# kasvii/GATOR

Hardware: AMD Instinct MI355X
Metric: meshes/sec (B=256, J=17) GATOR forward (higher is better)
Workload: dtype f32; 1 GPU; B=256 synthetic Human3.6M 17-joint poses per GPU, GAT+MDR forward fp32; batch_per_gpu=256, global_batch=256, num_joint=17, impl=fused, parallelism=dp1, mode=gather

## Files before the change

gator_amd/csrc/fused_api.hip:

```cpp
#include <hip/hip_runtime.h>

#include <algorithm>
#include <cmath>
#include <cstdlib>
#include <type_traits>
#include <vector>

#include "fused_state.h"
#include "x3_common.h"

namespace gator {
namespace {

static void graph_slot_free(FusedState::GraphSlot& g) {
    if (g.exec) (void)hipGraphExecDestroy((hipGraphExec_t)g.exec);
    if (g.graph) (void)hipGraphDestroy((hipGraph_t)g.graph);
    g.exec = g.graph = nullptr;
}
static void graphs_clear(FusedState* f) {
    for (auto& g : f->graphs) graph_slot_free(g);
    f->graphs.clear();
}
struct WsScope {
    FusedState* f; FusedWs* prev;
    WsScope(FusedState* f_, int i) : f(f_), prev(f_->ws) { f->ws = &f->sets[i]; }
    ~WsScope() { f->ws = prev; }
};

int fused_ensure_ws(gator_ctx* c, int B) {
    FusedState* f = c->fused;
    FusedWs& w = *f->ws;
    if (w.base && B <= w.cap) return GATOR_OK;
    if (w.base) {
        GATOR_HIP_CHECK(hipDeviceSynchronize());
        graphs_clear(f);
    }
    const int cap = B, MT = (cap + 31) / 32, J = c->J;
    const size_t tiles = (size_t)cap * kVT * 2 * kTile;
    size_t n = 0;
    auto layout = [&](float* block) {
        n = 0;
        auto region = [&](auto*& member, size_t floats) {
            if (block) member = reinterpret_cast<std::remove_reference_t<decltype(member)>>(block + n);
            n += (floats + 63) & ~(size_t)63;
        };
        region(w.vcp, (size_t)MT * 3 * kCB * kTile); region(w.vc, (size_t)cap * kV * 3);
        region(w.vf, 3 * tiles); region(w.q, 9 * tiles / 2); region(w.k, 9 * tiles / 2); region(w.v, 9 * tiles / 2);
        region(w.jkv, (size_t)cap * 12 * kTile); region(w.hf, (size_t)cap * kV * 32); region(w.lbf, (size_t)cap * kV * kE);
        region(w.feat, (size_t)cap * J * kC); region(w.vcp3, std::max(upsample_x3_vcp_elems(cap), upsample_x2_vcp_elems(cap)) / 2);
        region(w.lpart, gat_tail_part_floats(cap, J)); region(w.mdr_ctr, mdr_ctr_words(cap)); region(w.hpart, (size_t)cap * kVT * 128);
    };
    layout(nullptr);
    GATOR_TRY(w.base.alloc(n * sizeof(float)));
    GATOR_HIP_CHECK(hipMemset(w.base, 0, n * sizeof(float)));
    GATOR_HIP_CHECK(hipDeviceSynchronize());
    w.cap = cap;
    layout(w.base);
    return GATOR_OK;
}

std::vector<float> d2h(const float* p, size_t n) {
    std::vector<float> v(n);
    (void)hipMemcpy(v.data(), p, n * sizeof(float), hipMemcpyDeviceToHost);
    return v;
}

template <class F>
void fill_tile(float* dst, F tab) {
    for (int g = 0; g < 4; ++g)
        for (int lane = 0; lane < 64; ++lane)
            for (int j = 0; j < 4; ++j) dst[(g * 64 + lane) * 4 + j] = tab(lane & 31, 8 * g + 4 * (lane >> 5) + j);
}

int read_fused_options(const gator_ctx* c, FusedOptions* o) {
    auto flag = [](const char* name, bool dflt) { const char* e = getenv(name); return e ? atoi(e) != 0 : dflt; };
    auto num = [](const char* name, int dflt) { const char* e = getenv(name); return e ? atoi(e) : dflt; };
    auto set = [](const char* name) { return getenv(name) != nullptr; };
    const bool exact = c->arithmetic == GATOR_ARITH_EXACT_SPLIT;
    o->gat_x3 = flag("GATOR_GAT_X3", true);
    o->gat8 = o->gat_x3 && flag("GATOR_GAT8", true);
    o->gat8_h4 = !exact && flag("GATOR_GAT8_H4", true);
    o->gat8_lobyte = o->gat8 && o->gat8_h4 && flag("GATOR_GAT8_LOBYTE", true);
    o->gat_tiled_h4 = !exact && flag("GATOR_GAT_TILED_H4", true);
    o->gat_tiled = num("GATOR_GAT_TILED", -1);
    if (const int m = num("GATOR_GAT_TILED_MIN_BATCH", 0); m > 0) o->gat_tiled_min_batch = m;
    o->mdr_x3 = exact ? 1 : num("GATOR_MDR_X3", 2);
    o->up_x3 = exact ? 1 : num("GATOR_UPSAMPLE_X3", 2);
    if (c->parts & GATOR_PART_MDR) {
        if (o->up_x3 < 0 || o->up_x3 > 2) return fail(GATOR_EINVAL, "GATOR_UPSAMPLE_X3 must be 0, 1 or 2");
        if (o->mdr_x3 < 0 || o->mdr_x3 > 2) return fail(GATOR_EINVAL, "GATOR_MDR_X3 must be 0, 1 or 2");
    }
    o->gat8_tail = o->gat8 && o->gat8_h4 && o->mdr_x3 == 2 && flag("GATOR_GAT8_TAIL", true);
    o->mdr_persist = set("GATOR_MDR_PERSIST") ? flag("GATOR_MDR_PERSIST", false) : -1;
    o->mdr_persist_chunk = num("GATOR_MDR_PERSIST_CHUNK", 0);
    o->mdr_persist_grid = num("GATOR_MDR_PERSIST_GRID", 0);
    o->mdr_head_partials = flag("GATOR_MDR_HEAD_PARTIALS", true);
    o->c3_mdr = o->mdr_x3 == 2 && flag("GATOR_C3_MDR", true);
    o->c3_encoder = o->gat8 && o->gat8_h4 && o->gat_tiled_h4 && flag("GATOR_C3_ENCODER", true);
    o->c3_up_w1 = flag("GATOR_C3_UPSAMPLE_W1", true);
    o->c3_up_bf16 = o->up_x3 != 2 || flag("GATOR_C3_UPSAMPLE_BF16", false);
    o->c3_guard = flag("GATOR_C3_GUARD", true);
    o->graph = flag("GATOR_GRAPH", false);
    o->subbatch_streams = num("GATOR_SUBBATCH_STREAMS", 0);
#ifdef GATOR_DIAG
    o->gat8_dbg = num("GATOR_GAT8_DBG", 0);
    o->gat_stamps = set("GATOR_GAT_STAMPS");
    o->mdr_cut = num("GATOR_MDR_CUT", 0);
    o->mdr_stamps = set("GATOR_MDR_STAMPS");
    o->mdr_solo = set("GATOR_MDR_SOLO");
    o->mdr_ends = set("GATOR_MDR_ENDS");
#endif
    return GATOR_OK;
}

static double sym_eig_max(std::vector<double>& A, int n) {
    for (int sweep = 0; sweep < 64; ++sweep) {
        double off = 0, all = 0;
        for (int p = 0; p < n; ++p)
            for (int q = 0; q < n; ++q) { all += A[p * n + q] * A[p * n + q]; if (q > p) off += A[p * n + q] * A[p * n + q]; }
        if (!(off > 1e-30 * all)) break;
        for (int p = 0; p < n; ++p)
            for (int q = p + 1; q < n; ++q) {
                const double apq = A[p * n + q];
                if (apq == 0) continue;
                const double th = (A[q * n + q] - A[p * n + p]) / (2 * apq);
                const double t = (th >= 0 ? 1.0 : -1.0) / (std::fabs(th) + std::sqrt(th * th + 1));
                const double cs = 1 / std::sqrt(t * t + 1), sn = t * cs;
                for (int k = 0; k < n; ++k) {
                    const double kp = A[k * n + p], kq = A[k * n + q];
                    A[k * n + p] = cs * kp - sn * kq; A[k * n + q] = sn * kp + cs * kq;
                }
                for (int k = 0; k < n; ++k) {
                    const double pk = A[p * n + k], qk = A[q * n + k];
                    A[p * n + k] = cs * pk - sn * qk; A[q * n + k] = sn * pk + cs * qk;
                }
            }
    }
    double m = 0;
    for (int i = 0; i < n; ++i) m = std::max(m, A[i * n + i]);
    return m;
}

float c3_logit_bound(const Weights& w) {
    double worst = 0;
    for (int li = 0; li < 3; ++li) {
        const MdrLayerW& r = w.lay[li];
        const std::vector<float> wq = d2h(r.sa_w[0], 64 * 64), wk = d2h(r.sa_w[1], 64 * 64), bq = d2h(r.sa_b[0], 64), bk = d2h(r.sa_b[1], 64),
                                 a2 = d2h(r.a2, 64), b2 = d2h(r.b2, 64);
        double amax = 0, bn = 0;
        for (int i = 0; i < 64; ++i) { amax = std::max(amax, (double)std::fabs(a2[i])); bn += (double)b2[i] * b2[i]; }
        const double xn = amax * std::sqrt(63.0) + std::sqrt(bn);
        auto head_norm = [&](const std::vector<float>& W, const std::vector<float>& bias, int hd) {
            std::vector<double> G(32 * 32);
            double bb = 0;
            for (int i = 0; i < 32; ++i) {
                bb += (double)bias[32 * hd + i] * bias[32 * hd + i];
                for (int j = 0; j < 32; ++j) {
                    double acc = 0;
                    for (int k = 0; k < 64; ++k) acc += (double)W[(32 * hd + i) * 64 + k] * (double)W[(32 * hd + j) * 64 + k];
                    G[i * 32 + j] = acc;
                }
            }
            return std::sqrt(std::max(sym_eig_max(G, 32), 0.0)) * xn + std::sqrt(bb);
        };
        for (int hd = 0; hd < 2; ++hd)
            worst = std::max(worst, head_norm(wq, bq, hd) * head_norm(wk, bk, hd) / std::sqrt(32.0) * 1.4426950408889634);
    }
    return (float)worst;
}

struct PackItem { const float* src; int64_t wsn, wsk; int N, K; const float** dst; };
template <size_t n>
int pack_linears(const PackItem (&items)[n], float*& p, void* stream) {
    for (const PackItem& it : items) {
        GATOR_TRY(fused_pack_linear(it.src, it.wsn, it.wsk, it.N, it.K, p, stream));
        *it.dst = p;
        p += (size_t)nblk32(it.N) * nblk32(it.K) * kTile;
    }
    return GATOR_OK;
}

int fused_create_gat(gator_ctx* c, FusedState* f, void* stream) {
    const Weights& w = c->w;
    const int J = c->J;
    const size_t blk_tiles = 48 + 16 + 16 + 16 + 16 + 4 + 20 + 64 + 64 + 4 + 4 + 1 + 1;
    const size_t total = (kDepth * blk_tiles + 8 + 2 + 8 + 4 + 12) * kTile;
    GATOR_TRY(f->gbuf.alloc(total * sizeof(float)));
    float* p = f->gbuf;
    auto take = [&](size_t tiles) { float* r = p; p += tiles * kTile; return r; };
    std::vector<float> host;
    auto upload = [&](const std::vector<float>& v) -> const float* {
        float* d = take(v.size() / kTile);
        (void)hipMemcpy(d, v.data(), v.size() * sizeof(float), hipMemcpyHostToDevice);
        return d;
    };
    const std::vector<float> adiag = d2h(c->adj_diag, (size_t)kDepth * J), aoff = d2h(c->adj_off, (size_t)kDepth * J * J),
                             m1 = d2h(c->mask1, (size_t)J * J), m2 = d2h(c->mask2, (size_t)J * J), hb = d2h(c->hop_bias, (size_t)kH * J * J);
    for (int i = 0; i < kDepth; ++i) {
        const GatBlockW& r = w.blk[i];
        GatBlockPk& q = f->gblk[i];
        const PackItem items[] = {
            {r.qkv_w, 128, 1, 384, 128, &q.qkv}, {r.proj_w, 128, 1, 128, 128, &q.proj},
            {r.gcn_W, 1, 128, 128, 128, &q.w0}, {r.gcn_W + 128 * 128, 1, 128, 128, 128, &q.w1},
            {r.xl0_w, 128, 1, 128, 128, &q.lin0}, {r.xl1_w, 128, 1, 16, 128, &q.lin1}, {r.xlb_w, 144, 1, 128, 144, &q.back},
            {r.fc1_w, 128, 1, 512, 128, &q.fc1}, {r.fc2_w, 512, 1, 128, 512, &q.fc2}};
        GATOR_TRY(pack_linears(items, p, stream));
        const std::vector<float> M = d2h(r.gcn_M, (size_t)J * kC), b1 = d2h(r.xl1_b, 16);
        std::vector<float> mc(4 * kTile), md(4 * kTile);
        for (int nb = 0; nb < 4; ++nb) {
            for (int g = 0; g < 4; ++g)
                for (int lane = 0; lane < 64; ++lane)
                    for (int j = 0; j < 4; ++j) {
                        const int tok = 8 * g + 4 * (lane >> 5) + j, n = 32 * nb + (lane & 31);
                        mc[((nb * 4 + g) * 64 + lane) * 4 + j] = tok < J ? M[(size_t)tok * kC + n] : 0.f;
                    }
            fill_tile(md.data() + (size_t)nb * kTile, [&](int t, int ch) { return t < J ? adiag[i * J + t] * M[(size_t)t * kC + 32 * nb + ch] : 0.f; });
        }
        q.mc = upload(mc);
        q.mdT = upload(md);
        std::vector<float> t1(kTile), t2(kTile);
        fill_tile(t1.data(), [&](int t, int j) { return (t < J && j < J) ? aoff[((size_t)i * J + t) * J + j] : 0.f; });
        q.aoffT = upload(t1);
        fill_tile(t2.data(), [&](int t, int ch) {
            if (t >= J || ch >= 16) return 0.f;
            float deg = 0.f;
            for (int j = 0; j < J; ++j) deg += m2[(size_t)t * J + j];
            return deg * b1[ch];
        });
        q.f1b = upload(t2);
    }
    if (f->opt.gat_x3) {
        const int64_t ntiles = (p - f->gblk[0].qkv) / kTile;
        GATOR_TRY(f->gxbuf.alloc((size_t)ntiles * kTileX3 * sizeof(float)));
        int rc = fused_repack_x3(f->gblk[0].qkv, f->gxbuf, ntiles, stream);
        if (rc) return rc;
        if (f->opt.gat_tiled_h4) {
            float left = 0.f;
            GATOR_TRY(f->gxbuf_h3.alloc((size_t)ntiles * kTileX3 * sizeof(float)));
            rc = fused_repack_h3(f->gblk[0].qkv, f->gxbuf_h3, ntiles, &f->gat_tiled_wshift, &left, stream, (int64_t)blk_tiles, 264);
            if (rc == GATOR_OK && left > 1e-7f) rc = fail(GATOR_EUNSUPPORTED, "GAT weights span more than fp16 x 3 planes hold exactly: use GATOR_GAT_TILED_H4=0");
            if (rc) return rc;
        }
        if (f->opt.gat8) {
            rc = gat8_build_stream(f, stream);
            if (rc) return rc;
        }
    }
    std::vector<float> bt(8 * kTile), mt(kTile);
    for (int hd = 0; hd < kH; ++hd)
        fill_tile(bt.data() + (size_t)hd * kTile, [&](int t, int j) { return (t < J && j < J) ? hb[((size_t)hd * J + t) * J + j] : 0.f; });
    f->g_biasT = upload(bt);
    fill_tile(mt.data(), [&](int t, int j) { return (t < J && j < J) ? m1[(size_t)t * J + j] : 0.f; });
    f->g_m1T = upload(mt);
    fill_tile(mt.data(), [&](int t, int j) { return (t < J && j < J) ? m2[(size_t)t * J + j] : 0.f; });
    f->g_m2T = upload(mt);
    {
        std::vector<float> vv((size_t)kDepth * 2048);
        for (int i = 0; i < kDepth; ++i) {
            const GatBlockW& r = w.blk[i];
            const struct { const float* p; int n; } parts[] = {{r.n1w, 128}, {r.n1b, 128}, {r.qkv_b, 384}, {r.proj_b, 128}, {r.gcn_bias, 128},
                                                               {r.xl0_b, 128}, {r.xlb_b, 128}, {r.n2w, 128}, {r.n2b, 128}, {r.fc1_b, 512}, {r.fc2_b, 128}};
            size_t off = (size_t)i * 2048;
            for (auto& pt : parts) {
                const std::vector<float> h = d2h(pt.p, pt.n);
                std::copy(h.begin(), h.end(), vv.begin() + off);
                off += pt.n;
            }
        }
        f->g_vecs = upload(vv);
    }
    {
        float* dst = take(8);
        int rc = fused_pack_linear(w.gl3_W, 64, 1, 128, 64, dst, stream);
        if (rc) return rc;
        f->g_gl3 = dst;
        const std::vector<float> pe = d2h(c->pos_embed, (size_t)J * kC);
        std::vector<float> pt(4 * kTile);
        for (int kb = 0; kb < 4; ++kb)
            fill_tile(pt.data() + (size_t)kb * kTile, [&](int t, int ch) { return t < J ? pe[(size_t)t * kC + 32 * kb + ch] : 0.f; });
        f->g_posT = upload(pt);
    }
    {
        int rc = gat_prepare_device();
        if (rc == GATOR_OK) rc = gat_tiled_prepare_device();
        if (rc == GATOR_OK) rc = gat8_prepare_device();
        if (rc) return rc;
        hipDeviceProp_t prop;
        if (hipGetDeviceProperties(&prop, c->device) == hipSuccess && prop.multiProcessorCount > 0) f->n_cu = prop.multiProcessorCount;
    }
    GATOR_HIP_CHECK(hipStreamSynchronize((hipStream_t)stream));
    GATOR_HIP_CHECK(hipGetLastError());
    return GATOR_OK;
}

}

int fused_create(gator_ctx* c, void* stream) {
    if (c->impl == GATOR_IMPL_BASIC) return GATOR_OK;
    FusedState* f = new FusedState();
    c->fused = f;
    int rc = read_fused_options(c, &f->opt);
    if (rc) return rc;
    f->gat_tiled = f->opt.gat_tiled;
    f->graph_replay = f->opt.graph;
    const Weights& w = c->w;
    if (c->parts & GATOR_PART_GAT) {
        rc = fused_create_gat(c, f, stream);
        if (rc) return rc;
    }
    if (!(c->parts & GATOR_PART_MDR)) return GATOR_OK;
    if (f->opt.c3_mdr) {
        f->c3_logit_bound = c3_logit_bound(w);
        if (f->opt.c3_guard && !(f->c3_logit_bound <= 1024.0f)) f->opt.c3_mdr = f->opt.c3_encoder = false;
    }
    const size_t n_up = f->opt.up_x3 == 0 ? (size_t)3 * kOB * kCB * kTile : 0, n_layer = (size_t)64 * kTile;
    const size_t total = n_up + 3 * n_layer + 24 * kTile + 64 + (size_t)kVT * 2 * kTile + 3 * 64 + 1024;
    GATOR_TRY(f->wbuf.alloc(total * sizeof(float)));
    float* p = f->wbuf;
    auto take = [&](size_t k) { float* r = p; p += k; return r; };
    float* up = take(n_up);
    if (f->opt.up_x3 == 2) {
        GATOR_TRY(f->up_w2.alloc(upsample_x2_weight_elems() * 2));
        int rc = pack_upsample_x2(w.up_w, f->up_w2, &f->up_w2_unscale, stream);
        if (rc == GATOR_OK) rc = upsample_x2_prepare_device();
        if (rc) return rc;
    } else if (f->opt.up_x3 == 1) {
        GATOR_TRY(f->up_w3.alloc(upsample_x3_weight_elems() * 2));
        int rc = pack_upsample_x3(w.up_w, f->up_w3, stream);
        if (rc) return rc;
    } else {
        for (int tap = 0; tap < 3; ++tap) {
            int rc = fused_pack_linear(w.up_w + tap, (int64_t)kV * 3, 3, kNV, kV, up + (size_t)tap * kOB * kCB * kTile, stream);
            if (rc) return rc;
        }
        f->up_w = up;
    }
    for (int li = 0; li < 3; ++li) {
        const MdrLayerW& r = w.lay[li];
        MdrLayerP& q = f->lay[li];
        const PackItem items[] = {
            {r.wq, 64, 1, 64, 64, &q.wq}, {r.wk, 64, 1, 64, 64, &q.wk}, {r.wv, 64, 1, 64, 64, &q.wv}, {r.proj_w, 64, 1, 64, 64, &q.proj},
            {r.fc1_w, 64, 1, 256, 64, &q.fc1}, {r.fc2_w, 256, 1, 64, 256, &q.fc2},
            {r.sa_w[0], 64, 1, 64, 64, &q.sa[0]}, {r.sa_w[1], 64, 1, 64, 64, &q.sa[1]}, {r.sa_w[2], 64, 1, 64, 64, &q.sa[2]}, {r.sa_w[3], 64, 1, 64, 64, &q.sa[3]}};
        GATOR_TRY(pack_linears(items, p, stream));
    }
    {
        std::vector<float> hw(32 * 64, 0.f), hb(32, 0.f);
        const std::vector<float> mw = d2h(w.motion_w, 23 * 64), mb = d2h(w.motion_b, 23), bw = d2h(w.biasl_w, 3 * 64), bb = d2h(w.biasl_b, 3);
        for (int r = 0; r < 20; ++r) { std::copy(mw.begin() + r * 64, mw.begin() + (r + 1) * 64, hw.begin() + r * 64); hb[r] = mb[r]; }
        for (int r = 0; r < 3; ++r) {
            std::copy(bw.begin() + r * 64, bw.begin() + (r + 1) * 64, hw.begin() + (24 + r) * 64); hb[24 + r] = bb[r];
            std::copy(mw.begin() + (20 + r) * 64, mw.begin() + (21 + r) * 64, hw.begin() + (28 + r) * 64); hb[28 + r] = mb[20 + r];
        }
        if (c->alpha) {
            const std::vector<float> sw = d2h(w.scale_w, 64), sb = d2h(w.scale_b, 1);
            std::copy(sw.begin(), sw.end(), hw.begin() + 27 * 64);
            hb[27] = sb[0];
        }
        DevBuf<float> tmp;
        GATOR_TRY(tmp.alloc(hw.size() * sizeof(float)));
        GATOR_HIP_CHECK(hipMemcpy(tmp, hw.data(), hw.size() * sizeof(float), hipMemcpyHostToDevice));
        float* dst = take(2 * kTile);
        int rc = fused_pack_linear(tmp, 64, 1, 32, 64, dst, stream);
        GATOR_HIP_CHECK(hipStreamSynchronize((hipStream_t)stream));
        tmp.reset();
        if (rc) return rc;
        f->head_w = dst;
        if (f->opt.mdr_x3) {
            const int64_t ntiles = (dst + 2 * kTile - f->lay[0].wq) / kTile;
            GATOR_TRY(f->wxbuf.alloc((size_t)ntiles * kTileX3 * sizeof(float)));
            if (f->opt.mdr_x3 == 2) {
                float left = 0.f;
                rc = fused_repack_h3(f->lay[0].wq, f->wxbuf, ntiles, &f->mdr_wshift, &left, stream);
                if (rc == GATOR_OK && left > 1e-7f) rc = fail(GATOR_EUNSUPPORTED, "MDR weights span more than fp16 x 3 planes hold exactly (residual %.2e of the largest weight): use GATOR_MDR_X3=1", left);
            } else {
                rc = fused_repack_x3(f->lay[0].wq, f->wxbuf, ntiles, stream);
            }
            if (rc) return rc;
        }
        float* hbd = take(64);
        GATOR_HIP_CHECK(hipMemcpy(hbd, hb.data(), 32 * sizeof(float), hipMemcpyHostToDevice));
        f->head_b = hbd;
    }
    {
        float* dst = take(10 * kTile);
        int rc = fused_pack_linear(w.jfeat_w, 133, 1, 64, 133, dst, stream);
        if (rc) return rc;
        f->jfeat_p = dst;
        float* d128 = take(8 * kTile);
        rc = fused_pack_linear(w.jfeat_w + 5, 133, 1, 64, 128, d128, stream);
        if (rc) return rc;
        f->jfeat128_p = d128;
        if (f->opt.mdr_x3 == 2) {
            float left = 0.f;
// ... 359 lines not shown
```

gator_amd/csrc/fused_state.h:

```cpp
#pragma once
#include "internal.h"
#include <vector>

namespace gator {

constexpr int kVT = 14;
constexpr int kOB = 216;
constexpr int kCB = 14;
constexpr int kTile = 32 * 32;
constexpr int kMdrCtrChunks = 64;
__host__ __device__ inline size_t mdr_ctr_words(int B) { return (size_t)32 * kMdrCtrChunks + (size_t)4 * B; }

struct MdrLayerP {
    const float *wq, *wk, *wv, *proj, *fc1, *fc2, *sa[4];
};

struct GatBlockPk {
    const float *qkv, *proj, *w0, *w1, *lin0, *lin1, *back, *fc1, *fc2;
    const float *mc, *mdT, *aoffT, *f1b;
};

struct FusedWs {
    DevBuf<float> base;
    int cap = 0;
    float *vcp = nullptr;
    void* vcp3 = nullptr;
    float *vc = nullptr;
    float *vf = nullptr, *q = nullptr, *k = nullptr, *v = nullptr;
    float *jkv = nullptr;
    float *hf = nullptr;
    float *lbf = nullptr;
    float *feat = nullptr;
    float* hpart = nullptr;
    float *lpart = nullptr;
    bool mdr_ctr_clean = false;
    unsigned* mdr_ctr = nullptr;
    DevBuf<void> vcp16;
    int vcp16_cap = 0;
};

struct FusedOptions {
    bool gat_x3 = true;
    bool gat8 = true;
    bool gat8_h4 = true;
    bool gat8_lobyte = true;
    bool gat8_tail = true;
    bool gat_tiled_h4 = true;
    int gat_tiled = -1;
    int gat_tiled_min_batch = 1024;
    int mdr_x3 = 2;
    int up_x3 = 2;
    int mdr_persist = -1;
    int mdr_persist_chunk = 0;
    int mdr_persist_grid = 0;
    bool mdr_head_partials = true;
    bool c3_mdr = true;
    bool c3_encoder = true;
    bool c3_up_w1 = true;
    bool c3_up_bf16 = false;
    bool c3_guard = true;
    bool graph = false;
    int subbatch_streams = 0;
    int gat8_dbg = 0;
    bool gat_stamps = false;
    int mdr_cut = 0;
    bool mdr_stamps = false;
    bool mdr_solo = false;
    bool mdr_ends = false;
};

struct FusedState {
    ~FusedState();
    FusedOptions opt;
    DevBuf<float> wbuf;
    DevBuf<float> gbuf;
    GatBlockPk gblk[kDepth];
    const float *g_biasT = nullptr, *g_m1T = nullptr, *g_m2T = nullptr, *g_gl3 = nullptr, *g_posT = nullptr, *g_vecs = nullptr;
    const float* up_w = nullptr;
    DevBuf<void> up_w3;
    int gat_tiled = -1;
    int n_cu = 256;
    DevBuf<float> gxbuf;
    DevBuf<float> gxbuf_h3;
    int gat_tiled_wshift = 0;
    DevBuf<float> g8stream;
    DevBuf<float> g8stream_b;
    int gat8_wshift = 0;
    DevBuf<float> wxbuf;
    DevBuf<float> jf128_h3;
    int jf128_wshift = 0;
    int mdr_wshift = 0;
    float c3_logit_bound = 0.f;
    DevBuf<void> up_w2;
    float up_w2_unscale = 1.f;
    DevBuf<void> up_w16;
    DevBuf<void> jr_blk, jr_ent;
    DevBuf<float> jr_w;
    DevBuf<int> jr_rowptr;
    DevBuf<float> jr_P;
    int jr_nnz = 0, jr_nj = 0, jr_cap = 0;
    DevBuf<float> blk_tap;
    int blk_tap_cap = 0;
    MdrLayerP lay[3];
    const float* head_w = nullptr;
    const float* head_b = nullptr;
    const float* tok_base = nullptr;
    const float* tok_w3 = nullptr;
    struct GraphSlot {
        int B = 0; const void *in = nullptr, *verts = nullptr, *pose3d = nullptr; bool bf16 = false;
        int tiled = 0, persist = 0; const void* ws = nullptr;
        void *graph = nullptr, *exec = nullptr;
        unsigned long long used = 0;
    };
    static constexpr int kGraphSlots = 8;
    bool graph_replay = false;
    void* cap_stream = nullptr;
    std::vector<GraphSlot> graphs;
    unsigned long long graph_clock = 0, graph_launches = 0;
    FusedWs sets[2];
    FusedWs* ws = &sets[0];
    void* aux_stream = nullptr;
    void *ev_fork = nullptr, *ev_join = nullptr;
    const float* jfeat_p = nullptr;
    const float* jfeat5 = nullptr;
    const float* jfeat128_p = nullptr;
    const float* posj_T = nullptr;
};

int fused_pack_linear(const float* W, int64_t wsn, int64_t wsk, int N, int K, float* dst, void* stream);
inline int nblk32(int n) { return (n + 31) / 32; }
int launch_pack_vc(const float* vc, int B, float* vcp, void* stream);
int launch_upsample(const FusedState* f, const gator_ctx* c, int B, float* verts, void* stream);
int gat_prepare_device();
int gat_ensure_blk_tap(gator_ctx* c, FusedState* f, int B);
int launch_gat(gator_ctx* c, FusedState* f, const float* pose2d, int B, float* x_out, float* feat, void* stream, bool split_tail = false,
               int B_total = 0, int tap_row0 = 0, bool half16 = false, float* tail_jkv = nullptr);
int gat8_prepare_device();
int gat8_build_stream(FusedState* f, void* stream);
int launch_gat8(gator_ctx* c, FusedState* f, const float* pose2d, int B, float* feat, void* stream, int B_total = 0, int tap_row0 = 0, bool half16 = false,
                float* tail_x_out = nullptr, float* tail_jkv = nullptr, int ctr_B = 0);
bool gat8_tail_supported(const FusedState* f, bool half16);
int gat_tiled_prepare_device();
int gat_tiled_samples_per_wg(int J);
int launch_gat_tiled(gator_ctx* c, FusedState* f, const float* pose2d, int B, float* feat, void* stream, int B_total = 0, bool half16 = false);
size_t gat_tail_part_floats(int B, int J);
int launch_gat_tail(gator_ctx* c, FusedState* f, const float* pose2d, const float* feat, int B, float* x_out, void* stream, bool joint, bool zero_ctr = true);
size_t upsample_bf16_weight_elems();
size_t upsample_bf16_vcp_elems(int B);
int pack_upsample_bf16(const float* up_w, void* dst, void* stream);
int launch_upsample_bf16(const FusedState* f, const gator_ctx* c, const float* vc, int B, float* verts, void* stream);
size_t upsample_x3_weight_elems();
size_t upsample_x3_vcp_elems(int B);
int pack_upsample_x3(const float* up_w, void* dst, void* stream);
int launch_pack_vc_x3(const float* vc, int B, int cap, void* vcp3, void* stream);
int launch_upsample_x3(const FusedState* f, const gator_ctx* c, int B, float* verts, void* stream, bool with_joints = false);
int launch_jreg_reduce(const FusedState* f, int B, float* joints, void* stream);
size_t upsample_x2_weight_elems();
size_t upsample_x2_vcp_elems(int B);
int upsample_x2_prepare_device();
int pack_upsample_x2(const float* up_w, void* dst, float* unscale, void* stream);
int launch_pack_vc_x2(const float* vc, int B, void* vcp2, void* stream);
int launch_upsample_x2(const FusedState* f, const gator_ctx* c, int B, float* verts, void* stream, bool with_joints = false, bool w1 = false);
int launch_upsample_any(const FusedState* f, const gator_ctx* c, int B, float* verts, void* stream, bool with_joints = false, bool w1 = false);
int launch_mdr(gator_ctx* c, FusedState* f, const float* pc, int B, void* stream, const float* x_out = nullptr, const float* pose2d = nullptr, bool half16 = false);

}
```

gator_amd/csrc/upsample_x2.hip:

```cpp
#include <cmath>
#include <cstring>

#include "fused_common.h"
#include "fused_state.h"

namespace gator {
namespace {

typedef _Float16 f16x8 __attribute__((ext_vector_type(8)));
constexpr int kS16 = 28;
constexpr int kNBuf = 4, kStageFrags = 36;
constexpr int kActShift = 4;
#define GATOR_MFMA_F16(a, b, c) __builtin_amdgcn_mfma_f32_32x32x16_f16((a), (b), (c), 0, 0, 0)

__device__ __forceinline__ void split2(float x, _Float16& h, _Float16& l) {
    h = (_Float16)x;
    l = (_Float16)(x - (float)h);
}

__global__ void k_pack_up_x2(const float* __restrict__ w, _Float16* __restrict__ dst, int64_t n_frag_pairs, float scale) {
    const int64_t e = (int64_t)blockIdx.x * blockDim.x + threadIdx.x;
    if (e >= n_frag_pairs * 512) return;
    const int j = e & 7, lane = (e >> 3) & 63;
    int64_t r = e >> 9;
    const int tap = r % 3; r /= 3;
    const int o2 = r & 1; r >>= 1;
    const int s = r % kS16;
    const int op = (int)(r / kS16);
    const int o = 32 * (2 * op + o2) + (lane & 31), c = 16 * s + 8 * (lane >> 5) + j;
    const float x = (o < kNV && c < kV) ? w[((int64_t)o * kV + c) * 3 + tap] * scale : 0.f;
    _Float16 h, l;
    split2(x, h, l);
    const int64_t pair = (((int64_t)op * kS16 + s) * 2 + o2) * 3 + tap;
    dst[(pair * 2 + 0) * 512 + lane * 8 + j] = h;
    dst[(pair * 2 + 1) * 512 + lane * 8 + j] = l;
}
__global__ void k_pack_vc_x2(const float* __restrict__ vc, int B, _Float16* __restrict__ ap, int64_t n_frag_pairs) {
    const int64_t e = (int64_t)blockIdx.x * blockDim.x + threadIdx.x;
    if (e >= n_frag_pairs * 512) return;
    const int j = e & 7, lane = (e >> 3) & 63;
    int64_t r = e >> 9;
    const int lp = r % 3; r /= 3;
    const int mi = r & 3; r >>= 2;
    const int s = r % kS16;
    const int mg = (int)(r / kS16);
    const int smp = 32 * (4 * mg + mi) + (lane & 31), c = 16 * s + 8 * (lane >> 5) + j;
    const float x = (smp < B && c < kV) ? vc[((int64_t)smp * kV + c) * 3 + lp] * (float)(1 << kActShift) : 0.f;
    _Float16 h, l;
    split2(x, h, l);
    const int64_t pair = (((int64_t)mg * kS16 + s) * 4 + mi) * 3 + lp;
    ap[(pair * 2 + 0) * 512 + lane * 8 + j] = h;
    ap[(pair * 2 + 1) * 512 + lane * 8 + j] = l;
}

__global__ void k_absmax(const float* __restrict__ w, int64_t n, unsigned* __restrict__ out) {
    float m = 0.f;
    for (int64_t i = (int64_t)blockIdx.x * blockDim.x + threadIdx.x; i < n; i += (int64_t)gridDim.x * blockDim.x) {
        const float a = fabsf(w[i]);
        m = a > m || a != a ? a : m;
    }
    for (int o = 32; o > 0; o >>= 1) {
        const float q = __shfl_xor(m, o);
        m = q > m || q != q ? q : m;
    }
    if ((threadIdx.x & 63) == 0) atomicMax(out, __float_as_uint(m));
}

__device__ __forceinline__ void dma_frag(const void* base, unsigned lane_off, unsigned lds_dst) {
    unsigned keep;
    asm volatile("s_mov_b32 %0, m0\n\ts_mov_b32 m0, %3\n\ts_nop 0\n\tglobal_load_lds_dwordx4 %1, %2\n\ts_mov_b32 m0, %0"
                 : "=&s"(keep) : "v"(lane_off), "s"(base), "s"(lds_dst) : "memory");
}
template <int N> __device__ __forceinline__ void wait_vm() { asm volatile("s_waitcnt vmcnt(%0)" ::"n"(N) : "memory"); }

struct __attribute__((packed)) F3 { float x, y, z; };

struct JregEpi2 {
    const int2* blk;
    const int2* ent;
    const float* w;
    float* P;
    int nnz;
};

template <bool WLO = true>
__global__ __launch_bounds__(512, 1) void k_upsample_x2(const _Float16* __restrict__ ap, const _Float16* __restrict__ wp,
                                                        const float* __restrict__ bias, const float* __restrict__ tpl,
                                                        float* __restrict__ out, int B, int MT, int MG, int nwg, float unscale,
                                                        const JregEpi2 jr) {
    extern __shared__ __attribute__((aligned(16))) unsigned char lds_raw[];
    f16x8 (*st)[kStageFrags][64] = reinterpret_cast<f16x8 (*)[kStageFrags][64]>(lds_raw);
    const int lane = threadIdx.x & 63, wave = __builtin_amdgcn_readfirstlane(threadIdx.x >> 6);
    const int wg = xcd_remap(blockIdx.x, nwg);
    const int obp = wg / MG, mg = wg % MG;
    const int mi = wave & 3, oi = wave >> 2;
    const int ob = 2 * obp + oi, mt = 4 * mg + mi;
    const bool live = mt < MT;
    const unsigned lane_off = lane * 16;
    const unsigned lds0 = (unsigned)(unsigned long long)lds_raw;
    const char* a_src = reinterpret_cast<const char*>(ap) + (size_t)mg * kS16 * 24 * 1024;
    const char* w_src = reinterpret_cast<const char*>(wp) + (size_t)obp * kS16 * 12 * 1024;
    const char* src[5];
    unsigned stride[5], dsto[5];
#pragma unroll
    for (int i = 0; i < 5; ++i) {
        const int f = wave + 8 * i;
        src[i] = f < 24 ? a_src + f * 1024 : w_src + (f - 24) * 1024;
        stride[i] = f < 24 ? 24 * 1024 : 12 * 1024;
        dsto[i] = lds0 + f * 1024;
    }
    auto issue = [&](int s) {
        const unsigned dst = (unsigned)(s & (kNBuf - 1)) * kStageFrags * 1024;
#pragma unroll
        for (int i = 0; i < 4; ++i) dma_frag(src[i] + (size_t)s * stride[i], lane_off, dst + dsto[i]);
        if (wave < 4) dma_frag(src[4] + (size_t)s * stride[4], lane_off, dst + dsto[4]);
    };
    auto wait_landed = [&](int younger) {
        if (younger >= 1) { if (wave < 4) wait_vm<5>(); else wait_vm<4>(); }
        else wait_vm<0>();
    };
    f32x16 big[3], sm[3], tot[3];
#pragma unroll
    for (int l = 0; l < 3; ++l) { big[l] = zero16(); sm[l] = zero16(); tot[l] = zero16(); }
    f16x8 a[3][2], w[3][2];
    auto load_first = [&](int s) {
        const f16x8 (*cur)[64] = st[s & (kNBuf - 1)];
#pragma unroll
        for (int p = 0; p < 2; ++p) {
            a[0][p] = cur[mi * 6 + p][lane];
            w[0][p] = cur[24 + oi * 6 + p][lane];
            w[1][p] = cur[24 + oi * 6 + 2 + p][lane];
        }
    };
    auto load_rest = [&](int s) {
        const f16x8 (*cur)[64] = st[s & (kNBuf - 1)];
#pragma unroll
        for (int p = 0; p < 2; ++p) {
            a[1][p] = cur[mi * 6 + 2 + p][lane];
            w[2][p] = cur[24 + oi * 6 + 4 + p][lane];
            a[2][p] = cur[mi * 6 + 4 + p][lane];
        }
    };
    issue(0); issue(1); issue(2);
    if (wave < 4) wait_vm<10>(); else wait_vm<8>();
    __builtin_amdgcn_s_barrier();
    load_first(0);
#pragma unroll 1
    for (int s = 0; s < kS16; ++s) {
        if (s + 1 < kS16) wait_landed(kS16 - 2 - s);
        __builtin_amdgcn_s_barrier();
        if (s + 3 < kS16) issue(s + 3);
        load_rest(s);
        if (live) {
#pragma unroll
            for (int lp = 0; lp < 3; ++lp)
#pragma unroll
                for (int k = 2; k >= 0; --k) {
                    const int l = lp + 1 - k;
                    if (l < 0 || l > 2) continue;
                    big[l] = GATOR_MFMA_F16(a[lp][0], w[k][0], big[l]);
                    if constexpr (WLO) sm[l] = GATOR_MFMA_F16(a[lp][0], w[k][1], sm[l]);
                    sm[l] = GATOR_MFMA_F16(a[lp][1], w[k][0], sm[l]);
                }
            if (s % 7 == 6) {
#pragma unroll
                for (int l = 0; l < 3; ++l) { tot[l] += big[l]; big[l] = zero16(); }
            }
        }
        if (s + 1 < kS16) load_first(s + 1);
    }
    const int ov = 32 * ob + (lane & 31), h = lane >> 5;
    if (ov >= kNV || !live) return;
    const float bo = bias[ov];
    const float t0 = tpl[ov * 3], t1 = tpl[ov * 3 + 1], t2 = tpl[ov * 3 + 2];
    const int2 jb = jr.P ? jr.blk[ob] : int2{0, 0};
#pragma unroll
    for (int r = 0; r < 16; ++r) {
        const int smp = 32 * mt + kap(r) + 4 * h;
        if (smp < B) {
            F3 v;
            v.x = ((tot[0][r] + sm[0][r]) * unscale + bo) + t0;
            v.y = ((tot[1][r] + sm[1][r]) * unscale + bo) + t1;
            v.z = ((tot[2][r] + sm[2][r]) * unscale + bo) + t2;
            if (out) *reinterpret_cast<F3*>(out + ((int64_t)smp * kNV + ov) * 3) = v;
            for (int e = jb.x; e < jb.x + jb.y; ++e) {
                const int2 en = jr.ent[e];
                if (en.x == ov) {
                    const float we = jr.w[e];
                    F3 q;
                    q.x = we * v.x; q.y = we * v.y; q.z = we * v.z;
                    *reinterpret_cast<F3*>(jr.P + ((int64_t)smp * jr.nnz + en.y) * 3) = q;
                }
            }
        }
    }
}

constexpr size_t kX2Lds = (size_t)kNBuf * kStageFrags * 1024;

}

size_t upsample_x2_weight_elems() { return (size_t)(kOB / 2) * kS16 * 12 * 512; }
size_t upsample_x2_vcp_elems(int B) { return (size_t)((B + 127) / 128) * kS16 * 24 * 512; }

int upsample_x2_prepare_device() {
    GATOR_HIP_CHECK(hipFuncSetAttribute((const void*)k_upsample_x2<true>, hipFuncAttributeMaxDynamicSharedMemorySize, (int)kX2Lds));
    GATOR_HIP_CHECK(hipFuncSetAttribute((const void*)k_upsample_x2<false>, hipFuncAttributeMaxDynamicSharedMemorySize, (int)kX2Lds));
    return GATOR_OK;
}

int pack_upsample_x2(const float* up_w, void* dst, float* unscale, void* stream) {
    hipStream_t st = (hipStream_t)stream;
    DevBuf<unsigned> d_max;
    GATOR_TRY(d_max.alloc(sizeof(unsigned)));
    GATOR_HIP_CHECK(hipMemsetAsync(d_max, 0, sizeof(unsigned), st));
    const int64_t n = (int64_t)kNV * kV * 3;
    k_absmax<<<1024, 256, 0, st>>>(up_w, n, d_max.get());
    unsigned bits = 0;
    GATOR_HIP_CHECK(hipMemcpyAsync(&bits, d_max, sizeof(unsigned), hipMemcpyDeviceToHost, st));
    GATOR_HIP_CHECK(hipStreamSynchronize(st));
    d_max.reset();
    float wmax;
    static_assert(sizeof(wmax) == sizeof(bits), "float bits");
    memcpy(&wmax, &bits, sizeof(wmax));
    int shift = 0;
    if (wmax > 0.f && std::isfinite(wmax)) {
        int e;
        (void)std::frexp(wmax, &e);
        shift = 14 - e;
        if (shift > 24) shift = 24;
        if (shift < -16) shift = -16;
    }
    const int64_t pairs = (int64_t)upsample_x2_weight_elems() / 1024;
    k_pack_up_x2<<<(unsigned)((pairs * 512 + 255) / 256), 256, 0, st>>>(up_w, (_Float16*)dst, pairs, std::ldexp(1.0f, shift));
    GATOR_HIP_CHECK(hipGetLastError());
    *unscale = std::ldexp(1.0f, -(shift + kActShift));
    return GATOR_OK;
}

int launch_pack_vc_x2(const float* vc, int B, void* vcp2, void* stream) {
    const int64_t pairs = (int64_t)upsample_x2_vcp_elems(B) / 1024;
    k_pack_vc_x2<<<(unsigned)((pairs * 512 + 255) / 256), 256, 0, (hipStream_t)stream>>>(vc, B, (_Float16*)vcp2, pairs);
    GATOR_HIP_CHECK(hipGetLastError());
    return GATOR_OK;
}

int launch_upsample_x2(const FusedState* f, const gator_ctx* c, int B, float* verts, void* stream, bool with_joints, bool w1) {
    const int MT = (B + 31) / 32, MG = (MT + 3) / 4;
    JregEpi2 jr{};
    if (with_joints) { jr.blk = (const int2*)f->jr_blk.get(); jr.ent = (const int2*)f->jr_ent.get(); jr.w = f->jr_w.get(); jr.P = f->jr_P.get(); jr.nnz = f->jr_nnz; }
    const int nwg = (kOB / 2) * MG;
    if (w1) k_upsample_x2<false><<<nwg, 512, kX2Lds, (hipStream_t)stream>>>((const _Float16*)f->ws->vcp3, (const _Float16*)f->up_w2.get(), c->w.up_b, c->w.v6890,
                                                                           verts, B, MT, MG, nwg, f->up_w2_unscale, jr);
    else k_upsample_x2<true><<<nwg, 512, kX2Lds, (hipStream_t)stream>>>((const _Float16*)f->ws->vcp3, (const _Float16*)f->up_w2.get(), c->w.up_b, c->w.v6890,
                                                                       verts, B, MT, MG, nwg, f->up_w2_unscale, jr);
    GATOR_HIP_CHECK(hipGetLastError());
    return GATOR_OK;
}

}
```

Before: 418,000 meshes/sec.

## Add a finer-grained upsample kernel for the last batch tile group

Adds a second upsample GEMM kernel for the final group of up to four 32-sample M-tiles. It launches one workgroup per 32-vertex output block, with 192 threads per M-tile, its own DMA ring depth, and an LDS exchange that sums the three K-split partials in the epilogue. The original 512-thread kernel now only covers the full leading groups, which spreads work over more workgroups when the batch is small relative to CU count. The K loop also drops from 28 to 27 steps, apparently skipping a padded chunk, with a flush of the running partial sum on the last step. The cost is an extra kernel launch on the same stream and more template variants to maintain.

```diff
diff --git a/gator_amd/csrc/fused_api.hip b/gator_amd/csrc/fused_api.hip
--- a/gator_amd/csrc/fused_api.hip
+++ b/gator_amd/csrc/fused_api.hip
@@ -90,6 +90,8 @@
         if (o->up_x3 < 0 || o->up_x3 > 2) return fail(GATOR_EINVAL, "GATOR_UPSAMPLE_X3 must be 0, 1 or 2");
         if (o->mdr_x3 < 0 || o->mdr_x3 > 2) return fail(GATOR_EINVAL, "GATOR_MDR_X3 must be 0, 1 or 2");
     }
+    o->up_small = flag("GATOR_UPSAMPLE_SMALL", true);
+    if (const int t = num("GATOR_UPSAMPLE_SMALL_TILES", 0); t >= 1 && t <= 4) o->up_small_tiles = t;
     o->gat8_tail = o->gat8 && o->gat8_h4 && o->mdr_x3 == 2 && flag("GATOR_GAT8_TAIL", true);
     o->mdr_persist = set("GATOR_MDR_PERSIST") ? flag("GATOR_MDR_PERSIST", false) : -1;
     o->mdr_persist_chunk = num("GATOR_MDR_PERSIST_CHUNK", 0);
diff --git a/gator_amd/csrc/fused_state.h b/gator_amd/csrc/fused_state.h
--- a/gator_amd/csrc/fused_state.h
+++ b/gator_amd/csrc/fused_state.h
@@ -50,6 +50,8 @@
     int gat_tiled_min_batch = 1024;
     int mdr_x3 = 2;
     int up_x3 = 2;
+    bool up_small = true;
+    int up_small_tiles = 4;
     int mdr_persist = -1;
     int mdr_persist_chunk = 0;
     int mdr_persist_grid = 0;
diff --git a/gator_amd/csrc/upsample_x2.hip b/gator_amd/csrc/upsample_x2.hip
--- a/gator_amd/csrc/upsample_x2.hip
+++ b/gator_amd/csrc/upsample_x2.hip
@@ -1,5 +1,6 @@
 #include <cmath>
 #include <cstring>
+#include <type_traits>
 
 #include "fused_common.h"
 #include "fused_state.h"
@@ -9,6 +10,7 @@
 
 typedef _Float16 f16x8 __attribute__((ext_vector_type(8)));
 constexpr int kS16 = 28;
+constexpr int kSteps = 27;
 constexpr int kNBuf = 4, kStageFrags = 36;
 constexpr int kActShift = 4;
 #define GATOR_MFMA_F16(a, b, c) __builtin_amdgcn_mfma_f32_32x32x16_f16((a), (b), (c), 0, 0, 0)
@@ -82,6 +84,24 @@
     float* P;
     int nnz;
 };
+
+__device__ __forceinline__ void x2_finish_vertex(float s0, float s1, float s2, float unscale, float bo, float t0, float t1, float t2, float* __restrict__ out,
+                                                 const JregEpi2& jr, int2 jb, int smp, int ov) {
+    F3 v;
+    v.x = (s0 * unscale + bo) + t0;
+    v.y = (s1 * unscale + bo) + t1;
+    v.z = (s2 * unscale + bo) + t2;
+    if (out) *reinterpret_cast<F3*>(out + ((int64_t)smp * kNV + ov) * 3) = v;
+    for (int e = jb.x; e < jb.x + jb.y; ++e) {
+        const int2 en = jr.ent[e];
+        if (en.x == ov) {
+            const float we = jr.w[e];
+            F3 q;
+            q.x = we * v.x; q.y = we * v.y; q.z = we * v.z;
+            *reinterpret_cast<F3*>(jr.P + ((int64_t)smp * jr.nnz + en.y) * 3) = q;
+        }
+    }
+}
 
 template <bool WLO = true>
 __global__ __launch_bounds__(512, 1) void k_upsample_x2(const _Float16* __restrict__ ap, const _Float16* __restrict__ wp,
@@ -146,10 +166,10 @@
     __builtin_amdgcn_s_barrier();
     load_first(0);
 #pragma unroll 1
-    for (int s = 0; s < kS16; ++s) {
-        if (s + 1 < kS16) wait_landed(kS16 - 2 - s);
+    for (int s = 0; s < kSteps; ++s) {
+        if (s + 1 < kSteps) wait_landed(kSteps - 2 - s);
         __builtin_amdgcn_s_barrier();
-        if (s + 3 < kS16) issue(s + 3);
+        if (s + 3 < kSteps) issue(s + 3);
         load_rest(s);
         if (live) {
 #pragma unroll
@@ -162,12 +182,12 @@
                     if constexpr (WLO) sm[l] = GATOR_MFMA_F16(a[lp][0], w[k][1], sm[l]);
                     sm[l] = GATOR_MFMA_F16(a[lp][1], w[k][0], sm[l]);
                 }
-            if (s % 7 == 6) {
+            if (s % 7 == 6 || s == kSteps - 1) {
 #pragma unroll
                 for (int l = 0; l < 3; ++l) { tot[l] += big[l]; big[l] = zero16(); }
             }
         }
-        if (s + 1 < kS16) load_first(s + 1);
+        if (s + 1 < kSteps) load_first(s + 1);
     }
     const int ov = 32 * ob + (lane & 31), h = lane >> 5;
     if (ov >= kNV || !live) return;
@@ -177,26 +197,104 @@
 #pragma unroll
     for (int r = 0; r < 16; ++r) {
         const int smp = 32 * mt + kap(r) + 4 * h;
-        if (smp < B) {
-            F3 v;
-            v.x = ((tot[0][r] + sm[0][r]) * unscale + bo) + t0;
-            v.y = ((tot[1][r] + sm[1][r]) * unscale + bo) + t1;
-            v.z = ((tot[2][r] + sm[2][r]) * unscale + bo) + t2;
-            if (out) *reinterpret_cast<F3*>(out + ((int64_t)smp * kNV + ov) * 3) = v;
-            for (int e = jb.x; e < jb.x + jb.y; ++e) {
-                const int2 en = jr.ent[e];
-                if (en.x == ov) {
-                    const float we = jr.w[e];
-                    F3 q;
-                    q.x = we * v.x; q.y = we * v.y; q.z = we * v.z;
-                    *reinterpret_cast<F3*>(jr.P + ((int64_t)smp * jr.nnz + en.y) * 3) = q;
-                }
-            }
-        }
+        if (smp < B)
+            x2_finish_vertex(tot[0][r] + sm[0][r], tot[1][r] + sm[1][r], tot[2][r] + sm[2][r], unscale, bo, t0, t1, t2, out, jr, jb, smp, ov);
     }
 }
 
 constexpr size_t kX2Lds = (size_t)kNBuf * kStageFrags * 1024;
+
+constexpr int small_stages(int T) { return T <= 2 ? 8 : T == 3 ? 6 : 5; }
+constexpr int small_stage_frags(int T) { return 6 + 6 * T; }
+constexpr size_t small_lds(int T) { return (size_t)small_stages(T) * small_stage_frags(T) * 1024; }
+
+template <bool WLO, int T>
+__global__ __launch_bounds__(192 * T, 1) void k_upsample_x2_small(const _Float16* __restrict__ ap, const _Float16* __restrict__ wp,
+                                                                  const float* __restrict__ bias, const float* __restrict__ tpl,
+                                                                  float* __restrict__ out, int B, int mg, float unscale, const JregEpi2 jr) {
+    constexpr int NS = small_stages(T), AHEAD = NS - 1, SF = small_stage_frags(T);
+    constexpr int NW = T == 1 ? 2 : 1;
+    static_assert(AHEAD >= 2 && AHEAD <= kSteps && (2 + NW) * (AHEAD - 1) < 64, "ring depth / vmcnt range");
+    static_assert(T * 3 * 16 * 64 * sizeof(float) <= small_lds(T), "the epilogue's exchange fits the ring");
+    extern __shared__ __attribute__((aligned(16))) unsigned char lds_raw[];
+    const int lane = threadIdx.x & 63, wave = __builtin_amdgcn_readfirstlane(threadIdx.x >> 6);
+    const int ob = blockIdx.x;
+    const int ti = wave / 3, l = wave - 3 * ti;
+    const int mt = 4 * mg + ti;
+    const bool has_w = T <= 2 || wave < 6;
+    const unsigned lane_off = lane * 16;
+    const unsigned lds0 = (unsigned)(unsigned long long)lds_raw;
+    const int af = 6 + ti * 6 + l * 2, wf = T == 1 ? 2 * wave : wave;
+    const char* a_src = reinterpret_cast<const char*>(ap) + (((size_t)mg * kS16 * 4 + ti) * 6 + l * 2) * 1024;
+    const char* w_src = reinterpret_cast<const char*>(wp) + ((size_t)(ob >> 1) * kS16 * 2 + (ob & 1)) * 6 * 1024
+                        + (has_w ? wf : 0) * 1024;
+    auto issue = [&](int s) {
+        const unsigned dst = lds0 + (unsigned)(s % NS) * SF * 1024;
+        dma_frag(a_src + (size_t)s * 24 * 1024, lane_off, dst + af * 1024);
+        dma_frag(a_src + (size_t)s * 24 * 1024 + 1024, lane_off, dst + (af + 1) * 1024);
+        if (has_w) {
+#pragma unroll
+            for (int j = 0; j < NW; ++j) dma_frag(w_src + (size_t)s * 12 * 1024 + j * 1024, lane_off, dst + (wf + j) * 1024);
+        }
+    };
+    auto wait_landed = [&](auto K) {
+        if (has_w) wait_vm<(2 + NW) * decltype(K)::value>(); else wait_vm<2 * decltype(K)::value>();
+    };
+    const int lp0 = l == 2 ? 1 : 0, k0 = lp0 + 1 - l;
+    const bool three = l == 1;
+    f32x16 big = zero16(), sm = zero16(), tot = zero16();
+    f16x8 a[3][2], w[3][2];
+    auto frag = [&](int s, int f) -> const f16x8& {
+        return reinterpret_cast<const f16x8*>(lds_raw + (size_t)(s % NS) * SF * 1024 + (size_t)f * 1024)[lane];
+    };
+    auto load_pair = [&](int s, int j) {
+#pragma unroll
+        for (int p = 0; p < 2; ++p) {
+            a[j][p] = frag(s, 6 + ti * 6 + min(lp0 + j, 2) * 2 + p);
+            w[j][p] = frag(s, min(k0 + j, 2) * 2 + p);
+        }
+    };
+#pragma unroll
+    for (int s = 0; s < AHEAD; ++s) issue(s);
+    wait_landed(std::integral_constant<int, AHEAD - 1>());
+    __builtin_amdgcn_s_barrier();
+    load_pair(0, 0);
+#pragma unroll 1
+    for (int s = 0; s < kSteps; ++s) {
+        if (s + 1 < kSteps) {
+            if (s + AHEAD < kSteps + 1) wait_landed(std::integral_constant<int, AHEAD - 2>());
+            else wait_vm<0>();
+            __builtin_amdgcn_sched_barrier(0);
+            __builtin_amdgcn_s_barrier();
+            if (s + AHEAD < kSteps) issue(s + AHEAD);
+        }
+        load_pair(s, 1);
+        load_pair(s, 2);
+#pragma unroll
+        for (int j = 0; j < 3; ++j) {
+            if (j == 2 && !three) break;
+            big = GATOR_MFMA_F16(a[j][0], w[j][0], big);
+            if constexpr (WLO) sm = GATOR_MFMA_F16(a[j][0], w[j][1], sm);
+            sm = GATOR_MFMA_F16(a[j][1], w[j][0], sm);
+        }
+        if (s % 7 == 6 || s == kSteps - 1) { tot += big; big = zero16(); }
+        if (s + 1 < kSteps) load_pair(s + 1, 0);
+    }
+    float (*ex)[3][16][64] = reinterpret_cast<float (*)[3][16][64]>(lds_raw);
+    __syncthreads();
+#pragma unroll
+    for (int r = 0; r < 16; ++r) ex[ti][l][r][lane] = tot[r] + sm[r];
+    __syncthreads();
+    const int ov = 32 * ob + (lane & 31), h = lane >> 5;
+    if (ov >= kNV) return;
+    const float bo = bias[ov];
+    const float t0 = tpl[ov * 3], t1 = tpl[ov * 3 + 1], t2 = tpl[ov * 3 + 2];
+    const int2 jb = jr.P ? jr.blk[ob] : int2{0, 0};
+    for (int r = l; r < 16; r += 3) {
+        const int smp = 32 * mt + kap(r) + 4 * h;
+        if (smp < B) x2_finish_vertex(ex[ti][0][r][lane], ex[ti][1][r][lane], ex[ti][2][r][lane], unscale, bo, t0, t1, t2, out, jr, jb, smp, ov);
+    }
+}
 
 }
 
@@ -206,6 +304,11 @@
 int upsample_x2_prepare_device() {
     GATOR_HIP_CHECK(hipFuncSetAttribute((const void*)k_upsample_x2<true>, hipFuncAttributeMaxDynamicSharedMemorySize, (int)kX2Lds));
     GATOR_HIP_CHECK(hipFuncSetAttribute((const void*)k_upsample_x2<false>, hipFuncAttributeMaxDynamicSharedMemorySize, (int)kX2Lds));
+#define GATOR_X2_SMALL_LDS(T)                                                                                                                            \
+    GATOR_HIP_CHECK(hipFuncSetAttribute((const void*)k_upsample_x2_small<true, T>, hipFuncAttributeMaxDynamicSharedMemorySize, (int)small_lds(T)));      \
+    GATOR_HIP_CHECK(hipFuncSetAttribute((const void*)k_upsample_x2_small<false, T>, hipFuncAttributeMaxDynamicSharedMemorySize, (int)small_lds(T)));
+    GATOR_X2_SMALL_LDS(1) GATOR_X2_SMALL_LDS(2) GATOR_X2_SMALL_LDS(3) GATOR_X2_SMALL_LDS(4)
+#undef GATOR_X2_SMALL_LDS
     return GATOR_OK;
 }
 
@@ -245,16 +348,42 @@
     return GATOR_OK;
 }
 
+template <bool WLO, int T>
+static void launch_small(const FusedState* f, const gator_ctx* c, int B, int mg, float* verts, hipStream_t st, const JregEpi2& jr) {
+    k_upsample_x2_small<WLO, T><<<kOB, 192 * T, small_lds(T), st>>>((const _Float16*)f->ws->vcp3, (const _Float16*)f->up_w2.get(), c->w.up_b, c->w.v6890,
+                                                                     verts, B, mg, f->up_w2_unscale, jr);
+}
+
 int launch_upsample_x2(const FusedState* f, const gator_ctx* c, int B, float* verts, void* stream, bool with_joints, bool w1) {
     const int MT = (B + 31) / 32, MG = (MT + 3) / 4;
+    const hipStream_t st = (hipStream_t)stream;
     JregEpi2 jr{};
     if (with_joints) { jr.blk = (const int2*)f->jr_blk.get(); jr.ent = (const int2*)f->jr_ent.get(); jr.w = f->jr_w.get(); jr.P = f->jr_P.get(); jr.nnz = f->jr_nnz; }
-    const int nwg = (kOB / 2) * MG;
-    if (w1) k_upsample_x2<false><<<nwg, 512, kX2Lds, (hipStream_t)stream>>>((const _Float16*)f->ws->vcp3, (const _Float16*)f->up_w2.get(), c->w.up_b, c->w.v6890,
-                                                                           verts, B, MT, MG, nwg, f->up_w2_unscale, jr);
-    else k_upsample_x2<true><<<nwg, 512, kX2Lds, (hipStream_t)stream>>>((const _Float16*)f->ws->vcp3, (const _Float16*)f->up_w2.get(), c->w.up_b, c->w.v6890,
-                                                                       verts, B, MT, MG, nwg, f->up_w2_unscale, jr);
-    GATOR_HIP_CHECK(hipGetLastError());
+    const int T = MT - 4 * (MG - 1);
+    const bool small = f->opt.up_small && T <= f->opt.up_small_tiles;
+    const int big_groups = small ? MG - 1 : MG;
+    if (big_groups > 0) {
+        const int nwg = (kOB / 2) * big_groups;
+        if (w1) k_upsample_x2<false><<<nwg, 512, kX2Lds, st>>>((const _Float16*)f->ws->vcp3, (const _Float16*)f->up_w2.get(), c->w.up_b, c->w.v6890,
+                                                               verts, B, MT, big_groups, nwg, f->up_w2_unscale, jr);
+        else k_upsample_x2<true><<<nwg, 512, kX2Lds, st>>>((const _Float16*)f->ws->vcp3, (const _Float16*)f->up_w2.get(), c->w.up_b, c->w.v6890,
+                                                           verts, B, MT, big_groups, nwg, f->up_w2_unscale, jr);
+        GATOR_HIP_CHECK(hipGetLastError());
+    }
+    if (small) {
+        const int mg = MG - 1;
+        switch (2 * T + (w1 ? 1 : 0)) {
+            case 2: launch_small<true, 1>(f, c, B, mg, verts, st, jr); break;
+            case 3: launch_small<false, 1>(f, c, B, mg, verts, st, jr); break;
+            case 4: launch_small<true, 2>(f, c, B, mg, verts, st, jr); break;
+            case 5: launch_small<false, 2>(f, c, B, mg, verts, st, jr); break;
+            case 6: launch_small<true, 3>(f, c, B, mg, verts, st, jr); break;
+            case 7: launch_small<false, 3>(f, c, B, mg, verts, st, jr); break;
+            case 8: launch_small<true, 4>(f, c, B, mg, verts, st, jr); break;
+            default: launch_small<false, 4>(f, c, B, mg, verts, st, jr); break;
+        }
+        GATOR_HIP_CHECK(hipGetLastError());
+    }
     return GATOR_OK;
 }
 
```

New measurement: 406,700 meshes/sec. -2.7%, worse.
